# mvenouziou/Boosted_DETR

Hardware: AMD Instinct MI355X
Metric: images/sec training step (fwd+matcher+loss+bwd), 640x640 N=100 (higher is better)
Workload: dtype f32 (conv/GEMM products as 3 split-f16 [fwd] / split-bf16 [grad] MFMA products, f32 accumulate)

## Files before the change

boosted_detr_amd/csrc/attention.hip:

```cpp
#include "common.h"
#include "p16.h"
#include <stdlib.h>

namespace bdgemm { int gemm_mode(); }

namespace {

typedef unsigned int u32x4 __attribute__((ext_vector_type(4)));
typedef unsigned int u32x2 __attribute__((ext_vector_type(2)));
typedef short s16x4 __attribute__((ext_vector_type(4)));
typedef __bf16 abf16x8 __attribute__((ext_vector_type(8)));
typedef _Float16 af16x8 __attribute__((ext_vector_type(8)));
enum { AR_FP32 = 0, AR_BF16 = 1, AR_F16 = 2 };

constexpr int AD = 32;
constexpr int ALD = AD + 4;
constexpr int CH = 64;
constexpr int COLS_PER_BLOCK = 128;
#ifndef BDETR_ATTN_PF
#define BDETR_ATTN_PF 1
#endif
constexpr int APF = BDETR_ATTN_PF;

constexpr float LOG2E = 1.4426950408889634f, LN2 = 0.6931471805599453f;
__device__ __forceinline__ float exp2_fast(float x) { return __builtin_amdgcn_exp2f(x); }

__device__ __forceinline__ int crow(int e, int lh) { return (e & 3) + 8 * (e >> 2) + 4 * lh; }

struct ChunkRegs { f32x4 v[2]; };
__device__ __forceinline__ ChunkRegs fetch_chunk(const float* __restrict__ base, int64_t stride, int r0, int n) {
    ChunkRegs c;
#pragma unroll
    for (int p = 0; p < 2; ++p) {
        const int v = threadIdx.x + 256 * p;
        const int row = v >> 3, c4 = v & 7;
        const int rr = min(r0 + row, n - 1);
        f32x4 val = *reinterpret_cast<const f32x4*>(base + (int64_t)rr * stride + 4 * c4);
        if (r0 + row >= n) val = f32x4{0.f, 0.f, 0.f, 0.f};
        c.v[p] = val;
    }
    return c;
}
__device__ __forceinline__ void store_chunk(float* __restrict__ lds, const ChunkRegs& c) {
#pragma unroll
    for (int p = 0; p < 2; ++p) {
        const int v = threadIdx.x + 256 * p;
        *reinterpret_cast<f32x4*>(lds + (v >> 3) * ALD + 4 * (v & 7)) = c.v[p];
    }
}

__device__ __forceinline__ void load_col_regs(float (&r)[16], const float* __restrict__ base, int64_t stride, int col, bool ok, int lh) {
#pragma unroll
    for (int c = 0; c < 4; ++c) {
        f32x4 v = {0.f, 0.f, 0.f, 0.f};
        if (ok) v = *reinterpret_cast<const f32x4*>(base + (int64_t)col * stride + 16 * lh + 4 * c);
#pragma unroll
        for (int e = 0; e < 4; ++e) r[4 * c + e] = v[e];
    }
}

__device__ __forceinline__ f32x16 row_times_col(const float* __restrict__ sR, int t, const float (&creg)[16], int li, int lh) {
    f32x16 acc;
#pragma unroll
    for (int e = 0; e < 16; ++e) acc[e] = 0.f;
    f32x4 a[4];
#pragma unroll
    for (int c = 0; c < 4; ++c) a[c] = *reinterpret_cast<const f32x4*>(sR + (32 * t + li) * ALD + 16 * lh + 4 * c);
#pragma unroll
    for (int s = 0; s < 16; ++s) acc = __builtin_amdgcn_mfma_f32_32x32x2f32(a[s >> 2][s & 3], creg[s], acc, 0, 0, 0);
    return acc;
}

__device__ __forceinline__ void accumulate_rt_tile(f32x16& acc, const float* __restrict__ sR, int t, const f32x16& tile, int li, int lh) {
#pragma unroll
    for (int e = 0; e < 16; ++e) {
        const float a = sR[(32 * t + crow(e, lh)) * ALD + li];
        acc = __builtin_amdgcn_mfma_f32_32x32x2f32(a, tile[e], acc, 0, 0, 0);
    }
}

constexpr int IMG_PLANE = CH * 64, IMG_BYTES = 2 * IMG_PLANE;
constexpr int SMEM_BYTES = IMG_BYTES > CH * ALD * 4 ? IMG_BYTES : CH * ALD * 4;

template <int AR>
__device__ __forceinline__ void split2(float x0, float x1, unsigned& hi, unsigned& lo) {
    if (AR == AR_F16) p16_split2_f16(x0, x1, hi, lo); else p16_split2_bf16(x0, x1, hi, lo);
}
template <int AR>
__device__ __forceinline__ f32x16 mfma3(const u32x4& ah, const u32x4& al, const u32x4& bh, const u32x4& bl, f32x16 acc) {
    if (AR == AR_F16) {
#define H8(v) __builtin_bit_cast(af16x8, v)
        acc = __builtin_amdgcn_mfma_f32_32x32x16_f16(H8(al), H8(bh), acc, 0, 0, 0);
        acc = __builtin_amdgcn_mfma_f32_32x32x16_f16(H8(ah), H8(bl), acc, 0, 0, 0);
        acc = __builtin_amdgcn_mfma_f32_32x32x16_f16(H8(ah), H8(bh), acc, 0, 0, 0);
#undef H8
    } else {
#define B8(v) __builtin_bit_cast(abf16x8, v)
        acc = __builtin_amdgcn_mfma_f32_32x32x16_bf16(B8(al), B8(bh), acc, 0, 0, 0);
        acc = __builtin_amdgcn_mfma_f32_32x32x16_bf16(B8(ah), B8(bl), acc, 0, 0, 0);
        acc = __builtin_amdgcn_mfma_f32_32x32x16_bf16(B8(ah), B8(bh), acc, 0, 0, 0);
#undef B8
    }
    return acc;
}
template <int AR>
__device__ __forceinline__ void store_chunk_split(unsigned char* __restrict__ img, const ChunkRegs& c) {
#pragma unroll
    for (int p = 0; p < 2; ++p) {
        const int v = threadIdx.x + 256 * p, row = v >> 3, c4 = v & 7;
        unsigned h0, l0, h1, l1;
        split2<AR>(c.v[p][0], c.v[p][1], h0, l0);
        split2<AR>(c.v[p][2], c.v[p][3], h1, l1);
        const int off = row * 64 + (((c4 >> 1) ^ ((row >> 2) & 3)) << 4) + ((c4 & 1) << 3);
        *reinterpret_cast<u32x2*>(img + off) = u32x2{h0, h1};
        *reinterpret_cast<u32x2*>(img + IMG_PLANE + off) = u32x2{l0, l1};
    }
}
struct ColFrag { u32x4 h[2], l[2]; };
template <int AR>
__device__ __forceinline__ ColFrag col_frag(const float (&r)[16]) {
    ColFrag f;
#pragma unroll
    for (int s2 = 0; s2 < 2; ++s2)
#pragma unroll
        for (int e = 0; e < 4; ++e) { unsigned h, l; split2<AR>(r[8 * s2 + 2 * e], r[8 * s2 + 2 * e + 1], h, l); f.h[s2][e] = h; f.l[s2][e] = l; }
    return f;
}
template <int AR>
__device__ __forceinline__ f32x16 row_times_col_split(const unsigned char* __restrict__ img, int t, const ColFrag& c, int li, int lh) {
    f32x16 acc;
#pragma unroll
    for (int e = 0; e < 16; ++e) acc[e] = 0.f;
    const int row = 32 * t + li;
#pragma unroll
    for (int s2 = 0; s2 < 2; ++s2) {
        const int off = row * 64 + (((2 * lh + s2) ^ ((row >> 2) & 3)) << 4);
        const u32x4 ah = *reinterpret_cast<const u32x4*>(img + off), al = *reinterpret_cast<const u32x4*>(img + IMG_PLANE + off);
        acc = mfma3<AR>(ah, al, c.h[s2], c.l[s2], acc);
    }
    return acc;
}
template <int AR>
__device__ __forceinline__ void accumulate_rt_tile_split(f32x16& acc, const unsigned char* __restrict__ img, int t, const f32x16& tile, int lane) {
    const int lh = lane >> 5, g16 = (lane >> 4) & 1, q = (lane >> 2) & 3, p = lane & 3;
#pragma unroll
    for (int s2 = 0; s2 < 2; ++s2) {
        u32x4 bh, bl;
#pragma unroll
        for (int e = 0; e < 4; ++e) { unsigned h, l; split2<AR>(tile[8 * s2 + 2 * e], tile[8 * s2 + 2 * e + 1], h, l); bh[e] = h; bl[e] = l; }
        u32x2 ah2[2], al2[2];
#pragma unroll
        for (int jj = 0; jj < 2; ++jj) {
            const int row = 32 * t + 16 * s2 + 8 * jj + 4 * lh + q;
            const int off = row * 64 + ((((2 * g16) + (p >> 1)) ^ ((row >> 2) & 3)) << 4) + ((p & 1) << 3);
            ah2[jj] = __builtin_bit_cast(u32x2, __builtin_amdgcn_ds_read_tr16_b64_v4i16((__attribute__((address_space(3))) s16x4*)(img + off)));
            al2[jj] = __builtin_bit_cast(u32x2, __builtin_amdgcn_ds_read_tr16_b64_v4i16((__attribute__((address_space(3))) s16x4*)(img + IMG_PLANE + off)));
        }
        const u32x4 ah = {ah2[0][0], ah2[0][1], ah2[1][0], ah2[1][1]}, al = {al2[0][0], al2[0][1], al2[1][0], al2[1][1]};
        acc = mfma3<AR>(ah, al, bh, bl, acc);
    }
}

template <int AR> struct ColOperand { float r[16]; ColFrag f; };
template <int AR>
__device__ __forceinline__ void chunk_store(unsigned char* smem, const ChunkRegs& c) {
    if constexpr (AR == AR_FP32) store_chunk(reinterpret_cast<float*>(smem), c); else store_chunk_split<AR>(smem, c);
}
template <int AR>
__device__ __forceinline__ f32x16 rows_x_col(const unsigned char* smem, int t, const ColOperand<AR>& c, int li, int lh) {
    if constexpr (AR == AR_FP32) return row_times_col(reinterpret_cast<const float*>(smem), t, c.r, li, lh);
    else return row_times_col_split<AR>(smem, t, c.f, li, lh);
}
template <int AR>
__device__ __forceinline__ void rowsT_x_tile(f32x16& acc, const unsigned char* smem, int t, const f32x16& tile, int lane) {
    if constexpr (AR == AR_FP32) accumulate_rt_tile(acc, reinterpret_cast<const float*>(smem), t, tile, lane & 31, lane >> 5);
    else accumulate_rt_tile_split<AR>(acc, smem, t, tile, lane);
}
template <int AR>
__device__ __forceinline__ void col_operand(ColOperand<AR>& c, const float* __restrict__ base, int64_t stride, int col, bool ok, int lh) {
    load_col_regs(c.r, base, stride, col, ok, lh);
    if constexpr (AR != AR_FP32) c.f = col_frag<AR>(c.r);
}

template <int AR>
__global__ __launch_bounds__(256) void attn_fwd_kernel(const float* __restrict__ q, const float* __restrict__ k, const float* __restrict__ v,
                                                       float* __restrict__ o, float* __restrict__ lse,
                                                       int h, int nq, int nk, float scale) {
    __shared__ __attribute__((aligned(16))) unsigned char sK[SMEM_BYTES];
    __shared__ __attribute__((aligned(16))) unsigned char sV[SMEM_BYTES];
    const int b = blockIdx.z, head = blockIdx.y;
    const int lane = threadIdx.x & 63, wave = threadIdx.x >> 6, li = lane & 31, lh = lane >> 5;
    const int64_t D = (int64_t)h * AD;
    const int qi = blockIdx.x * COLS_PER_BLOCK + wave * 32 + li;
    const bool qok = qi < nq;
    ColOperand<AR> qr;
    col_operand<AR>(qr, q + (int64_t)b * nq * D + head * AD, D, qi, qok, lh);
    const float* kbase = k + (int64_t)b * nk * D + head * AD;
    const float* vbase = v + (int64_t)b * nk * D + head * AD;

    f32x16 oacc;
#pragma unroll
    for (int e = 0; e < 16; ++e) oacc[e] = 0.f;
    float m = -INFINITY, l = 0.f;

    const float scale2 = scale * LOG2E;
    const bool wave_active = blockIdx.x * COLS_PER_BLOCK + wave * 32 < nq;
    ChunkRegs ck[APF], cv[APF];
#pragma unroll
    for (int p = 0; p < APF; ++p) {
        ck[p] = ChunkRegs{}; cv[p] = ChunkRegs{};
        if (p * CH < nk) { ck[p] = fetch_chunk(kbase, D, p * CH, nk); cv[p] = fetch_chunk(vbase, D, p * CH, nk); }
    }
    for (int c0 = 0; c0 < nk; c0 += CH) {
        __syncthreads();
        chunk_store<AR>(sK, ck[0]);
        chunk_store<AR>(sV, cv[0]);
        __syncthreads();
#pragma unroll
        for (int p = 0; p + 1 < APF; ++p) { ck[p] = ck[p + 1]; cv[p] = cv[p + 1]; }
        if (c0 + APF * CH < nk) { ck[APF - 1] = fetch_chunk(kbase, D, c0 + APF * CH, nk); cv[APF - 1] = fetch_chunk(vbase, D, c0 + APF * CH, nk); }
        if (!wave_active) continue;
        f32x16 s[2];
        float cmax = -INFINITY;
        const bool full = c0 + CH <= nk;
#pragma unroll
        for (int t = 0; t < 2; ++t) {
            s[t] = rows_x_col<AR>(sK, t, qr, li, lh);
#pragma unroll
            for (int e = 0; e < 16; ++e) s[t][e] *= scale2;
        }
        if (!full) {
#pragma unroll
            for (int t = 0; t < 2; ++t)
#pragma unroll
                for (int e = 0; e < 16; ++e) if (!(c0 + 32 * t + crow(e, lh) < nk)) s[t][e] = -INFINITY;
        }
#pragma unroll
        for (int t = 0; t < 2; ++t)
#pragma unroll
            for (int e = 0; e < 16; ++e) cmax = fmaxf(cmax, s[t][e]);
        cmax = fmaxf(cmax, __shfl_xor(cmax, 32, 64));
        const float mn = fmaxf(m, cmax);
        const float alpha = exp2_fast(m - mn);
        float psum = 0.f;
#pragma unroll
        for (int t = 0; t < 2; ++t)
#pragma unroll
            for (int e = 0; e < 16; ++e) { const float p = exp2_fast(s[t][e] - mn); s[t][e] = p; psum += p; }
        psum += __shfl_xor(psum, 32, 64);
        l = l * alpha + psum;
        m = mn;
#pragma unroll
        for (int e = 0; e < 16; ++e) oacc[e] *= alpha;
#pragma unroll
        for (int t = 0; t < 2; ++t) rowsT_x_tile<AR>(oacc, sV, t, s[t], lane);
    }
    if (qok) {
        const float inv = 1.0f / l;
        float* orow = o + (((int64_t)b * h + head) * nq + qi) * AD;
#pragma unroll
        for (int e = 0; e < 16; ++e) orow[crow(e, lh)] = oacc[e] * inv;
        if (lh == 0) lse[((int64_t)b * h + head) * nq + qi] = m * LN2 + logf(l);
    }
}

__global__ __launch_bounds__(256) void attn_dvec_kernel(const float* __restrict__ o, const float* __restrict__ d_o, float* __restrict__ dvec, int64_t rows) {
    const int64_t row = ((int64_t)blockIdx.x * 256 + threadIdx.x) >> 3;
    const int c4 = threadIdx.x & 7;
    float s = 0.f;
    if (row < rows) {
        const f32x4 a = reinterpret_cast<const f32x4*>(o)[row * 8 + c4], g = reinterpret_cast<const f32x4*>(d_o)[row * 8 + c4];
        s = a[0] * g[0] + a[1] * g[1] + a[2] * g[2] + a[3] * g[3];
    }
    s += __shfl_xor(s, 1, 64); s += __shfl_xor(s, 2, 64); s += __shfl_xor(s, 4, 64);
    if (row < rows && c4 == 0) dvec[row] = s;
}

template <bool KCOL, int AR>
__global__ __launch_bounds__(256) void attn_bwd_kernel(const float* __restrict__ q, const float* __restrict__ k, const float* __restrict__ v,
                                                       const float* __restrict__ d_o, const float* __restrict__ lse, const float* __restrict__ dvec,
                                                       float* __restrict__ out1, float* __restrict__ out2,
                                                       int h, int nq, int nk, float scale) {
    __shared__ __attribute__((aligned(16))) unsigned char sR1[SMEM_BYTES];
    __shared__ __attribute__((aligned(16))) unsigned char sR2[SMEM_BYTES];
    __shared__ float sL[CH], sD[CH];
    const int b = blockIdx.z, head = blockIdx.y;
    const int lane = threadIdx.x & 63, wave = threadIdx.x >> 6, li = lane & 31, lh = lane >> 5;
    const int64_t D = (int64_t)h * AD;
    const int ncol = KCOL ? nk : nq, nrow = KCOL ? nq : nk;
    const int ci = blockIdx.x * COLS_PER_BLOCK + wave * 32 + li;
    const bool cok = ci < ncol;
    const int64_t bh = (int64_t)b * h + head;

    const float* c1base = (KCOL ? k : q) + (int64_t)b * ncol * D + head * AD;
    const float* c2base = KCOL ? (v + (int64_t)b * nk * D + head * AD) : (d_o + bh * nq * AD);
    const int64_t c2stride = KCOL ? D : AD;
    ColOperand<AR> c1r, c2r;
    col_operand<AR>(c1r, c1base, D, ci, cok, lh);
    col_operand<AR>(c2r, c2base, c2stride, ci, cok, lh);
    const float* r1base = (KCOL ? q : k) + (int64_t)b * nrow * D + head * AD;
    const float* r2base = KCOL ? (d_o + bh * nq * AD) : (v + (int64_t)b * nk * D + head * AD);
    const int64_t r2stride = KCOL ? AD : D;

    float Lcol = 0.f, Dcol = 0.f;
    if (!KCOL && cok) { Lcol = lse[bh * nq + ci] * LOG2E; Dcol = dvec[bh * nq + ci]; }
    const float scale2 = scale * LOG2E;

    f32x16 acc1, acc2;
#pragma unroll
    for (int e = 0; e < 16; ++e) { acc1[e] = 0.f; acc2[e] = 0.f; }

    const bool wave_active = blockIdx.x * COLS_PER_BLOCK + wave * 32 < ncol;
    ChunkRegs c1[APF], c2[APF];
#pragma unroll
    for (int p = 0; p < APF; ++p) {
        c1[p] = ChunkRegs{}; c2[p] = ChunkRegs{};
        if (p * CH < nrow) { c1[p] = fetch_chunk(r1base, D, p * CH, nrow); c2[p] = fetch_chunk(r2base, r2stride, p * CH, nrow); }
    }
    for (int c0 = 0; c0 < nrow; c0 += CH) {
        __syncthreads();
        chunk_store<AR>(sR1, c1[0]);
        chunk_store<AR>(sR2, c2[0]);
        if (KCOL && threadIdx.x < CH) {
            const int qi = c0 + threadIdx.x;
            sL[threadIdx.x] = qi < nq ? lse[bh * nq + qi] * LOG2E : 0.f;
            sD[threadIdx.x] = qi < nq ? dvec[bh * nq + qi] : 0.f;
        }
        __syncthreads();
#pragma unroll
        for (int p = 0; p + 1 < APF; ++p) { c1[p] = c1[p + 1]; c2[p] = c2[p + 1]; }
        if (c0 + APF * CH < nrow) { c1[APF - 1] = fetch_chunk(r1base, D, c0 + APF * CH, nrow); c2[APF - 1] = fetch_chunk(r2base, r2stride, c0 + APF * CH, nrow); }
        if (!wave_active) continue;
        const bool full = c0 + CH <= nrow;
#pragma unroll
        for (int t = 0; t < 2; ++t) {
            f32x16 S = rows_x_col<AR>(sR1, t, c1r, li, lh);
            f32x16 G = rows_x_col<AR>(sR2, t, c2r, li, lh);
#pragma unroll
            for (int e = 0; e < 16; ++e) {
                const int r = 32 * t + crow(e, lh);
                const float Lq = KCOL ? sL[r] : Lcol, Dq = KCOL ? sD[r] : Dcol;
                const float p = (full || c0 + r < nrow) ? exp2_fast(S[e] * scale2 - Lq) : 0.f;
                S[e] = p * (G[e] - Dq) * scale;
                G[e] = p;
            }
            rowsT_x_tile<AR>(acc1, sR1, t, S, lane);
            if (KCOL) rowsT_x_tile<AR>(acc2, sR2, t, G, lane);
        }
    }
    if (cok) {
        float* o1 = out1 + ((int64_t)b * ncol + ci) * D + head * AD;
#pragma unroll
        for (int e = 0; e < 16; ++e) o1[crow(e, lh)] = acc1[e];
        if (KCOL) {
            float* o2 = out2 + ((int64_t)b * ncol + ci) * D + head * AD;
#pragma unroll
            for (int e = 0; e < 16; ++e) o2[crow(e, lh)] = acc2[e];
        }
    }
}

bool attn_split_enabled() {
    static int on = -1;
    if (on < 0) { const char* e = getenv("BDETR_ATTN_SPLIT"); on = e ? atoi(e) != 0 : 1; }
    return on != 0;
}

int check_attn(const void* a, const void* b, const void* c, int B, int h, int nq, int nk, const char* who) {
    BDETR_CHECK_ARG(a && b && c, "%s: null pointer", who);
    BDETR_CHECK_ARG(B > 0 && h > 0 && nq > 0 && nk > 0 && B <= 65535 && h <= 65535, "%s: bad sizes B=%d h=%d nq=%d nk=%d", who, B, h, nq, nk);
    BDETR_CHECK_ARG(((uintptr_t)a & 15) == 0 && ((uintptr_t)b & 15) == 0 && ((uintptr_t)c & 15) == 0, "%s: operands must be 16-byte aligned", who);
    return 0;
}

}

extern "C" int bdetr_attention_head_dim(void) { return AD; }

extern "C" int bdetr_attention_fwd(const float* q, const float* k, const float* v, float* o, float* lse,
                                   int B, int h, int nq, int nk, float scale, void* stream) {
    if (int e = check_attn(q, k, v, B, h, nq, nk, "bdetr_attention_fwd")) return e;
    BDETR_CHECK_ARG(o && lse, "bdetr_attention_fwd: null output");
    dim3 grid((nq + COLS_PER_BLOCK - 1) / COLS_PER_BLOCK, h, B);
    const int mode = attn_split_enabled() ? bdgemm::gemm_mode() : BDETR_GEMM_FP32;
    if (mode == BDETR_GEMM_SPLIT) hipLaunchKernelGGL((attn_fwd_kernel<AR_F16>), grid, dim3(256), 0, (hipStream_t)stream, q, k, v, o, lse, h, nq, nk, scale);
    else if (mode == BDETR_GEMM_BF16X3) hipLaunchKernelGGL((attn_fwd_kernel<AR_BF16>), grid, dim3(256), 0, (hipStream_t)stream, q, k, v, o, lse, h, nq, nk, scale);
    else hipLaunchKernelGGL((attn_fwd_kernel<AR_FP32>), grid, dim3(256), 0, (hipStream_t)stream, q, k, v, o, lse, h, nq, nk, scale);
    return bdetr_launch_status("attention_fwd");
}

extern "C" int bdetr_attention_bwd(const float* q, const float* k, const float* v, const float* o, const float* d_o,
                                   const float* lse, float* dq, float* dk, float* dv, float* dvec_ws,
                                   int B, int h, int nq, int nk, float scale, void* stream) {
    if (int e = check_attn(q, k, v, B, h, nq, nk, "bdetr_attention_bwd")) return e;
    BDETR_CHECK_ARG(o && d_o && lse && dq && dk && dv && dvec_ws, "bdetr_attention_bwd: null pointer");
    hipStream_t st = (hipStream_t)stream;
    const int64_t rows = (int64_t)B * h * nq;
    hipLaunchKernelGGL(attn_dvec_kernel, dim3((unsigned)((rows * 8 + 255) / 256)), dim3(256), 0, st, o, d_o, dvec_ws, rows);
    const dim3 gq((nq + COLS_PER_BLOCK - 1) / COLS_PER_BLOCK, h, B), gk((nk + COLS_PER_BLOCK - 1) / COLS_PER_BLOCK, h, B);
    if (!attn_split_enabled() || bdgemm::gemm_mode() == BDETR_GEMM_FP32 || bdgemm::gemm_mode() == BDETR_GEMM_BF16X6) {
        hipLaunchKernelGGL((attn_bwd_kernel<false, AR_FP32>), gq, dim3(256), 0, st, q, k, v, d_o, lse, dvec_ws, dq, (float*)nullptr, h, nq, nk, scale);
        hipLaunchKernelGGL((attn_bwd_kernel<true, AR_FP32>), gk, dim3(256), 0, st, q, k, v, d_o, lse, dvec_ws, dk, dv, h, nq, nk, scale);
    } else {
        hipLaunchKernelGGL((attn_bwd_kernel<false, AR_BF16>), gq, dim3(256), 0, st, q, k, v, d_o, lse, dvec_ws, dq, (float*)nullptr, h, nq, nk, scale);
        hipLaunchKernelGGL((attn_bwd_kernel<true, AR_BF16>), gk, dim3(256), 0, st, q, k, v, d_o, lse, dvec_ws, dk, dv, h, nq, nk, scale);
    }
    return bdetr_launch_status("attention_bwd");
}
```

Measured before the change: 654.9.

## Fuse attention backward dvec, dQ and dK/dV kernels into one launch

Merges the separate row-dot (dvec) kernel and the two backward attention kernels into one fused launch, whose grid covers both the key-column and query-column blocks. Each block recomputes the o·dO row dot products it needs locally: the dQ path computes them for its own query rows into shared memory, and the dK/dV path computes them per streamed chunk from prefetched o rows. This removes two kernel launches and the dvec round trip through global memory, and lets the dQ and dK/dV work run concurrently. The cost is redundant dot-product work and extra o loads per chunk in the dK/dV path, plus more register pressure from the additional prefetch buffer.

```diff
diff --git a/boosted_detr_amd/csrc/attention.hip b/boosted_detr_amd/csrc/attention.hip
--- a/boosted_detr_amd/csrc/attention.hip
+++ b/boosted_detr_amd/csrc/attention.hip
@@ -264,31 +264,32 @@
     }
 }
 
+__device__ __forceinline__ float row_dot8(const f32x4& a, const f32x4& g) {
+#pragma clang fp contract(off)
+    float s = a[0] * g[0] + a[1] * g[1] + a[2] * g[2] + a[3] * g[3];
+    s += __shfl_xor(s, 1, 64); s += __shfl_xor(s, 2, 64); s += __shfl_xor(s, 4, 64);
+    return s;
+}
+
 __global__ __launch_bounds__(256) void attn_dvec_kernel(const float* __restrict__ o, const float* __restrict__ d_o, float* __restrict__ dvec, int64_t rows) {
     const int64_t row = ((int64_t)blockIdx.x * 256 + threadIdx.x) >> 3;
     const int c4 = threadIdx.x & 7;
-    float s = 0.f;
-    if (row < rows) {
-        const f32x4 a = reinterpret_cast<const f32x4*>(o)[row * 8 + c4], g = reinterpret_cast<const f32x4*>(d_o)[row * 8 + c4];
-        s = a[0] * g[0] + a[1] * g[1] + a[2] * g[2] + a[3] * g[3];
-    }
-    s += __shfl_xor(s, 1, 64); s += __shfl_xor(s, 2, 64); s += __shfl_xor(s, 4, 64);
+    f32x4 a = {0.f, 0.f, 0.f, 0.f}, g = a;
+    if (row < rows) { a = reinterpret_cast<const f32x4*>(o)[row * 8 + c4]; g = reinterpret_cast<const f32x4*>(d_o)[row * 8 + c4]; }
+    const float s = row_dot8(a, g);
     if (row < rows && c4 == 0) dvec[row] = s;
 }
 
-template <bool KCOL, int AR>
-__global__ __launch_bounds__(256) void attn_bwd_kernel(const float* __restrict__ q, const float* __restrict__ k, const float* __restrict__ v,
-                                                       const float* __restrict__ d_o, const float* __restrict__ lse, const float* __restrict__ dvec,
-                                                       float* __restrict__ out1, float* __restrict__ out2,
-                                                       int h, int nq, int nk, float scale) {
-    __shared__ __attribute__((aligned(16))) unsigned char sR1[SMEM_BYTES];
-    __shared__ __attribute__((aligned(16))) unsigned char sR2[SMEM_BYTES];
-    __shared__ float sL[CH], sD[CH];
+template <bool KCOL, int AR, bool DOT>
+__device__ __forceinline__ void attn_bwd_block(const float* __restrict__ q, const float* __restrict__ k, const float* __restrict__ v, const float* __restrict__ o,
+                                               const float* __restrict__ d_o, const float* __restrict__ lse, const float* __restrict__ dvec,
+                                               float* __restrict__ out1, float* __restrict__ out2, int h, int nq, int nk, float scale, int bx,
+                                               unsigned char* sR1, unsigned char* sR2, float* sL, float* sD) {
     const int b = blockIdx.z, head = blockIdx.y;
     const int lane = threadIdx.x & 63, wave = threadIdx.x >> 6, li = lane & 31, lh = lane >> 5;
     const int64_t D = (int64_t)h * AD;
     const int ncol = KCOL ? nk : nq, nrow = KCOL ? nq : nk;
-    const int ci = blockIdx.x * COLS_PER_BLOCK + wave * 32 + li;
+    const int ci = bx * COLS_PER_BLOCK + wave * 32 + li;
     const bool cok = ci < ncol;
     const int64_t bh = (int64_t)b * h + head;
 
@@ -303,19 +304,37 @@
     const int64_t r2stride = KCOL ? AD : D;
 
     float Lcol = 0.f, Dcol = 0.f;
-    if (!KCOL && cok) { Lcol = lse[bh * nq + ci] * LOG2E; Dcol = dvec[bh * nq + ci]; }
+    if (!KCOL && cok) { Lcol = lse[bh * nq + ci] * LOG2E; if (!DOT) Dcol = dvec[bh * nq + ci]; }
+    const float* orows = DOT ? o + bh * nq * AD : nullptr;
+    if (!KCOL && DOT) {
+        float* sDot = reinterpret_cast<float*>(sR1);
+#pragma unroll
+        for (int p = 0; p < COLS_PER_BLOCK / 32; ++p) {
+            const int rl = 32 * p + (threadIdx.x >> 3), row = bx * COLS_PER_BLOCK + rl, c4 = threadIdx.x & 7;
+            const int64_t off = (int64_t)min(row, nq - 1) * AD + 4 * c4;
+            f32x4 a = *reinterpret_cast<const f32x4*>(orows + off), g = *reinterpret_cast<const f32x4*>(d_o + bh * nq * AD + off);
+            if (row >= nq) { a = f32x4{0.f, 0.f, 0.f, 0.f}; g = a; }
+            const float s = row_dot8(a, g);
+            if (c4 == 0) sDot[rl] = s;
+        }
+        __syncthreads();
+        Dcol = sDot[wave * 32 + li];
+    }
     const float scale2 = scale * LOG2E;
 
     f32x16 acc1, acc2;
 #pragma unroll
     for (int e = 0; e < 16; ++e) { acc1[e] = 0.f; acc2[e] = 0.f; }
 
-    const bool wave_active = blockIdx.x * COLS_PER_BLOCK + wave * 32 < ncol;
-    ChunkRegs c1[APF], c2[APF];
+    const bool wave_active = bx * COLS_PER_BLOCK + wave * 32 < ncol;
+    ChunkRegs c1[APF], c2[APF], co[KCOL && DOT ? APF : 1];
 #pragma unroll
     for (int p = 0; p < APF; ++p) {
-        c1[p] = ChunkRegs{}; c2[p] = ChunkRegs{};
-        if (p * CH < nrow) { c1[p] = fetch_chunk(r1base, D, p * CH, nrow); c2[p] = fetch_chunk(r2base, r2stride, p * CH, nrow); }
+        c1[p] = ChunkRegs{}; c2[p] = ChunkRegs{}; if (KCOL && DOT) co[p] = ChunkRegs{};
+        if (p * CH < nrow) {
+            c1[p] = fetch_chunk(r1base, D, p * CH, nrow); c2[p] = fetch_chunk(r2base, r2stride, p * CH, nrow);
+            if (KCOL && DOT) co[p] = fetch_chunk(orows, AD, p * CH, nrow);
+        }
     }
     for (int c0 = 0; c0 < nrow; c0 += CH) {
         __syncthreads();
@@ -324,12 +343,23 @@
         if (KCOL && threadIdx.x < CH) {
             const int qi = c0 + threadIdx.x;
             sL[threadIdx.x] = qi < nq ? lse[bh * nq + qi] * LOG2E : 0.f;
-            sD[threadIdx.x] = qi < nq ? dvec[bh * nq + qi] : 0.f;
+            if (!DOT) sD[threadIdx.x] = qi < nq ? dvec[bh * nq + qi] : 0.f;
+        }
+        if (KCOL && DOT) {
+#pragma unroll
+            for (int p = 0; p < 2; ++p) {
+                const int vv = threadIdx.x + 256 * p;
+                const float s = row_dot8(co[0].v[p], c2[0].v[p]);
+                if ((vv & 7) == 0) sD[vv >> 3] = s;
+            }
         }
         __syncthreads();
 #pragma unroll
-        for (int p = 0; p + 1 < APF; ++p) { c1[p] = c1[p + 1]; c2[p] = c2[p + 1]; }
-        if (c0 + APF * CH < nrow) { c1[APF - 1] = fetch_chunk(r1base, D, c0 + APF * CH, nrow); c2[APF - 1] = fetch_chunk(r2base, r2stride, c0 + APF * CH, nrow); }
+        for (int p = 0; p + 1 < APF; ++p) { c1[p] = c1[p + 1]; c2[p] = c2[p + 1]; if (KCOL && DOT) co[p] = co[p + 1]; }
+        if (c0 + APF * CH < nrow) {
+            c1[APF - 1] = fetch_chunk(r1base, D, c0 + APF * CH, nrow); c2[APF - 1] = fetch_chunk(r2base, r2stride, c0 + APF * CH, nrow);
+            if (KCOL && DOT) co[APF - 1] = fetch_chunk(orows, AD, c0 + APF * CH, nrow);
+        }
         if (!wave_active) continue;
         const bool full = c0 + CH <= nrow;
 #pragma unroll
@@ -358,6 +388,36 @@
             for (int e = 0; e < 16; ++e) o2[crow(e, lh)] = acc2[e];
         }
     }
+}
+
+template <bool KCOL, int AR>
+__global__ __launch_bounds__(256) void attn_bwd_kernel(const float* __restrict__ q, const float* __restrict__ k, const float* __restrict__ v,
+                                                       const float* __restrict__ d_o, const float* __restrict__ lse, const float* __restrict__ dvec,
+                                                       float* __restrict__ out1, float* __restrict__ out2,
+                                                       int h, int nq, int nk, float scale) {
+    __shared__ __attribute__((aligned(16))) unsigned char sR1[SMEM_BYTES];
+    __shared__ __attribute__((aligned(16))) unsigned char sR2[SMEM_BYTES];
+    __shared__ float sL[CH], sD[CH];
+    attn_bwd_block<KCOL, AR, false>(q, k, v, nullptr, d_o, lse, dvec, out1, out2, h, nq, nk, scale, blockIdx.x, sR1, sR2, sL, sD);
+}
+
+template <int AR>
+__global__ __launch_bounds__(256) void attn_bwd_fused_kernel(const float* __restrict__ q, const float* __restrict__ k, const float* __restrict__ v,
+                                                             const float* __restrict__ o, const float* __restrict__ d_o, const float* __restrict__ lse,
+                                                             float* __restrict__ dq, float* __restrict__ dk, float* __restrict__ dv,
+                                                             int h, int nq, int nk, float scale, int gk) {
+    __shared__ __attribute__((aligned(16))) unsigned char sR1[SMEM_BYTES];
+    __shared__ __attribute__((aligned(16))) unsigned char sR2[SMEM_BYTES];
+    __shared__ float sL[CH], sD[CH];
+    const int bx = (blockIdx.x + blockIdx.y) % gridDim.x;
+    if (bx < gk) attn_bwd_block<true, AR, true>(q, k, v, o, d_o, lse, nullptr, dk, dv, h, nq, nk, scale, bx, sR1, sR2, sL, sD);
+    else attn_bwd_block<false, AR, true>(q, k, v, o, d_o, lse, nullptr, dq, nullptr, h, nq, nk, scale, bx - gk, sR1, sR2, sL, sD);
+}
+
+bool attn_bwd_fused_enabled() {
+    static int on = -1;
+    if (on < 0) { const char* e = getenv("BDETR_ATTN_BWD_FUSED"); on = e ? atoi(e) != 0 : 1; }
+    return on != 0;
 }
 
 bool attn_split_enabled() {
@@ -396,9 +456,17 @@
     BDETR_CHECK_ARG(o && d_o && lse && dq && dk && dv && dvec_ws, "bdetr_attention_bwd: null pointer");
     hipStream_t st = (hipStream_t)stream;
     const int64_t rows = (int64_t)B * h * nq;
+    const int nbq = (nq + COLS_PER_BLOCK - 1) / COLS_PER_BLOCK, nbk = (nk + COLS_PER_BLOCK - 1) / COLS_PER_BLOCK;
+    const bool exact = !attn_split_enabled() || bdgemm::gemm_mode() == BDETR_GEMM_FP32 || bdgemm::gemm_mode() == BDETR_GEMM_BF16X6;
+    if (attn_bwd_fused_enabled()) {
+        const dim3 gf(nbk + nbq, h, B);
+        if (exact) hipLaunchKernelGGL((attn_bwd_fused_kernel<AR_FP32>), gf, dim3(256), 0, st, q, k, v, o, d_o, lse, dq, dk, dv, h, nq, nk, scale, nbk);
+        else hipLaunchKernelGGL((attn_bwd_fused_kernel<AR_BF16>), gf, dim3(256), 0, st, q, k, v, o, d_o, lse, dq, dk, dv, h, nq, nk, scale, nbk);
+        return bdetr_launch_status("attention_bwd");
+    }
     hipLaunchKernelGGL(attn_dvec_kernel, dim3((unsigned)((rows * 8 + 255) / 256)), dim3(256), 0, st, o, d_o, dvec_ws, rows);
-    const dim3 gq((nq + COLS_PER_BLOCK - 1) / COLS_PER_BLOCK, h, B), gk((nk + COLS_PER_BLOCK - 1) / COLS_PER_BLOCK, h, B);
-    if (!attn_split_enabled() || bdgemm::gemm_mode() == BDETR_GEMM_FP32 || bdgemm::gemm_mode() == BDETR_GEMM_BF16X6) {
+    const dim3 gq(nbq, h, B), gk(nbk, h, B);
+    if (exact) {
         hipLaunchKernelGGL((attn_bwd_kernel<false, AR_FP32>), gq, dim3(256), 0, st, q, k, v, d_o, lse, dvec_ws, dq, (float*)nullptr, h, nq, nk, scale);
         hipLaunchKernelGGL((attn_bwd_kernel<true, AR_FP32>), gk, dim3(256), 0, st, q, k, v, d_o, lse, dvec_ws, dk, dv, h, nq, nk, scale);
     } else {
```

Result: no change. 661.2 (median of 6 runs) (+1.0%).
